# gkm2708/gym-lmaze

Hardware: AMD Instinct MI355X
Metric: env steps/sec (whole node), 1M parallel 11x11 mazes at 1/2/4/8 MI355X (higher is better)
Workload: dtype int32

## Files before the change

### gym-lmaze_amd/csrc/lmaze_foveal.hip

```cpp
#include <cstdio>
#include <cstring>
#include <type_traits>

#include "lmaze_common.h"
#include "lmaze_visit.h"

#ifdef LMAZE_EXPERIMENT
#define LMAZE_WARM_V4(args) ((((args).p.launch_hint >> 16) & 1024) != 0)
#define LMAZE_XP(args, mask) ((((args).p.launch_hint >> 16) & (mask)) != 0)
#else
#define LMAZE_WARM_V4(args) false
#define LMAZE_XP(args, mask) false
#endif

namespace lmaze {

constexpr int FOV = LMAZE_FOVEA;
constexpr int W25 = FOV * FOV;

enum FovealMode { FM_STEP = 0, FM_RESET = 1, FM_SETGOAL = 2, FM_PLANNER = 3 };

struct FovealArgs {
    LmazeFovealParams p;
    LmazeFovealBuffers b;
    const uint8_t* layouts;
    const int32_t* action;
    const int32_t* goal2;
    const uint8_t* mask;
    int64_t n;
    int32_t place;
    uint64_t seed, epoch;
    int64_t env_base;
    const uint64_t* epoch_in;
    uint64_t* epoch_out;
    int32_t nt;
    int32_t auto_reset;
    LaunchInfo* info;
};

struct FovealRoll {
    int32_t T;
    float* reward_t;
    uint8_t* done_t;
    float* freward_t;
    uint8_t* fdone_t;
};

struct FovealRollObs : FovealRoll {
    float* obs_t;
    float* obs_local_t;
    int32_t every;
};

__device__ __forceinline__ float* roll_slot(const FovealRoll&, int64_t, int64_t, int, int) { return nullptr; }
__device__ __forceinline__ float* roll_slot(const FovealRollObs& ro, int64_t n, int64_t base, int t, int per) {
    if (ro.obs_t == nullptr || (t + 1) % ro.every != 0) return nullptr;
    return ro.obs_t + ((size_t)((t + 1) / ro.every - 1) * n + base) * per;
}
__device__ __forceinline__ float* roll_lslot(const FovealRoll&, int64_t, int64_t, int) { return nullptr; }
__device__ __forceinline__ float* roll_lslot(const FovealRollObs& ro, int64_t n, int64_t base, int t) {
    if (ro.obs_local_t == nullptr || (t + 1) % ro.every != 0) return nullptr;
    return ro.obs_local_t + ((size_t)((t + 1) / ro.every - 1) * n + base) * (4 * W25);
}
__device__ __forceinline__ void roll_store4(const FovealRoll&, float4*, const float*) {}
__device__ __forceinline__ void roll_store4(const FovealRollObs&, float4* p, const float* v) {
    *p = make_float4(v[0], v[1], v[2], v[3]);
}

struct EnvRec {
    int16_t cx, cy;
    int16_t px, py;
    int16_t gx, gy;
    int16_t lid;
    int16_t action;
    int32_t skip;
    int32_t flat;
    int16_t b0x, b0y;
    int16_t b1x, b1y;
    int16_t f1x, f1y;
    int16_t upd;
    int16_t pad;
};


template <int U>
__device__ __forceinline__ void mask_counts(const uint64_t* goal_rows, const uint64_t* ball_rows, int G, int& cg, int& cb) {
    cg = 0; cb = 0;
#pragma unroll U
    for (int x = 1; x <= G - 2; ++x) { cg += __popcll(goal_rows[x]); cb += __popcll(ball_rows[x]); }
}

template <int U>
__device__ __forceinline__ int mask_kth(const uint64_t* rows, int G, int k, int hole) {
    int xr = -1, kk = 0, acc = 0;
#pragma unroll U
    for (int x = 1; x <= G - 2; ++x) {
        uint64_t m = rows[x];
        const unsigned hy = (unsigned)(hole - x * G);
        if (hy < (unsigned)G) m &= ~(1ull << hy);
        const int c = __popcll(m);
        if (xr < 0 && k < acc + c) { xr = x; kk = k - acc; }
        acc += c;
    }
    if (xr < 0) return -1;
    uint64_t m = rows[xr];
    const unsigned hy = (unsigned)(hole - xr * G);
    if (hy < (unsigned)G) m &= ~(1ull << hy);
    uint32_t h = (uint32_t)m;
    int base = 0;
    const int cl = __popc(h);
    if (kk >= cl) { kk -= cl; h = (uint32_t)(m >> 32); base = 32; }
    for (; kk > 0; --kk) h &= h - 1;
    return xr * G + base + (__ffs((int)h) - 1);
}

template <int U>
__device__ __forceinline__ void place_goal_ball(const uint64_t* goal_rows, const uint64_t* ball_rows, int G, uint4 d,
                                                int& goal_cell, int& ball_cell) {
    goal_cell = -1;
    ball_cell = -1;
    int cg, cb;
    mask_counts<U>(goal_rows, ball_rows, G, cg, cb);
    if (cg > 0) goal_cell = mask_kth<U>(goal_rows, G, (int)__umulhi(d.x, (uint32_t)cg), -1);
    if (goal_cell >= 0 && ((ball_rows[goal_cell / G] >> (goal_cell % G)) & 1ull)) --cb;
    if (cb > 0) ball_cell = mask_kth<U>(ball_rows, G, (int)__umulhi(d.y, (uint32_t)cb), goal_cell);
}

__device__ __forceinline__ int wrap5(int i) {
    if (i >= 0 && i < FOV) return i;
    if (i < 0 && i >= -FOV) return i + FOV;
    return -1;
}

__device__ __forceinline__ uint32_t window_bits(const uint64_t* rows, int G, int cx, int cy) {
    uint32_t m = 0;
    const int y0 = cy - 2;
#pragma unroll
    for (int i = 0; i < FOV; ++i) {
        const int x = cx - 2 + i;
        const uint64_t b = (x >= 0 && x < G) ? rows[x] : 0ull;
        const uint32_t w = (uint32_t)(y0 >= 0 ? (b >> y0) : (b << -y0)) & 31u;
        m |= w << (FOV * i);
    }
    return m;
}

__device__ __forceinline__ uint32_t onehot_bits(int tx, int ty, int cx, int cy) {
    const int i = tx - cx + 2, j = ty - cy + 2;
    return (i >= 0 && i < FOV && j >= 0 && j < FOV) ? (1u << (FOV * i + j)) : 0u;
}

__device__ __forceinline__ void put_bits(uint32_t* bits, int off, uint32_t m) {
    const int w = off >> 5, sh = off & 31;
    atomicOr(&bits[w], m << sh);
    if (sh > 32 - W25) atomicOr(&bits[w + 1], m >> (32 - sh));
}

__device__ __forceinline__ void lds_dma16(const uint32_t* src, uint32_t* lds_wave_base) {
    typedef __attribute__((address_space(1))) void gvoid;
    typedef __attribute__((address_space(3))) void lvoid;
    __builtin_amdgcn_global_load_lds((gvoid*)src, (lvoid*)lds_wave_base, 16, 0, 0);
}

__device__ __forceinline__ void nibble_floats(const uint32_t* bits, int q, float (&v)[4]) {
    const uint32_t nib = bits[q >> 3] >> ((q & 7) << 2);
#pragma unroll
    for (int k = 0; k < 4; ++k) v[k] = __uint_as_float((0u - ((nib >> k) & 1u)) & 0x3f800000u);
}

constexpr int VISIT_BIAS = LMAZE_VISIT_BIAS, VISIT_RENORM = LMAZE_VISIT_RENORM;
constexpr int VT = 4;
constexpr int VPC = 28;
__host__ __device__ __forceinline__ int visit_tag(int x, int y) { return 0x100 | ((x & 0x7f) << 9) | ((y & 0x7f) << 16); }

__host__ __device__ __forceinline__ int visit_tiles(int G) { return (G + VT - 1) / VT; }
__device__ __forceinline__ uint32_t visit_true(uint32_t bits, int E) { return lmaze_visit_true(bits, E); }
__device__ __forceinline__ uint32_t visit_add(uint32_t bits, int E) { return lmaze_visit_add(bits, E); }

#ifndef LMAZE_WIN_SUB
// ... 137 lines not shown
        const int row = rem / S, col = rem - row * S;
        const float* r0 = src + p * PC + (row / ET) * GT;
        const int k0 = col / ET;
        const float v0 = r0[k0], v1 = r0[k0 + 1];
        int row1 = row + 1, p1 = p;
        if (row1 == S) { row1 = 0; ++p1; }
        const float vw = src[p1 * PC + (row1 / ET) * GT];
        const int edge = (k0 + 1) * ET;
        float v[4];
#pragma unroll
        for (int j = 0; j < 4; ++j) {
            const int cj = col + j;
            v[j] = cj >= S ? vw : (cj >= edge ? v1 : v0);
        }
        const int count = len - (q << 2);
        if (count >= 4) {
            if (NT) {
                typedef float f4 __attribute__((ext_vector_type(4)));
                f4 t = {v[0], v[1], v[2], v[3]};
                stream_store16(reinterpret_cast<f4*>(dst) + q, t);
            } else {
                reinterpret_cast<float4*>(dst)[q] = make_float4(v[0], v[1], v[2], v[3]);
            }
        } else {
            for (int j = 0; j < count; ++j) dst[(q << 2) + j] = v[j];
        }
    }
}

constexpr size_t kFovealStreamBytes = (size_t)192 << 20;

static size_t lds_limit() {
    static size_t limit = 0;
    if (limit == 0) {
        int dev = 0, v = 0;
        if (hipGetDevice(&dev) == hipSuccess && hipDeviceGetAttribute(&v, hipDeviceAttributeMaxSharedMemoryPerBlock, dev) == hipSuccess && v > 0)
            limit = (size_t)v;
        else
            limit = 64 * 1024;
    }
    return limit;
}

template <int VARIANT>
static size_t foveal_lds(const LmazeFovealParams& p, int epb) {
    const int cells = p.grid * p.grid;
    const int L = VARIANT == LMAZE_VARIANT_V1 ? 1 : p.n_layouts;
    size_t lds = (size_t)epb * 64 + (3 * (size_t)L * p.grid + 2 * (size_t)p.grid) * 8 + (size_t)((L * cells + 15) & ~15);
    if (VARIANT == LMAZE_VARIANT_V4 || VARIANT == LMAZE_VARIANT_V5)
        lds += (size_t)epb * (2 * W25 * 4 + 8);
    return lds;
}

static size_t lds_for_cap(size_t lds, int per_cu) {
    if (per_cu >= 1 && per_cu <= 8) {
        const size_t cap = 160 * 1024;
        const size_t want = ((cap / per_cu + cap / (per_cu + 1)) / 2) & ~(size_t)255;
        if (want > lds && want <= lds_limit()) return want;
    }
    return lds;
}

template <int VARIANT, int MODE, int EPB>
static hipError_t launch_foveal_one(const FovealArgs& a, hipStream_t s) {
    size_t lds = foveal_lds<VARIANT>(a.p, EPB);
    if constexpr (EPB > 32) {
        if (lds > lds_limit()) return launch_foveal_one<VARIANT, MODE, EPB / 2>(a, s);
    }
    const int64_t nchunks = (a.n + EPB - 1) / EPB;
    const int m = MODE == FM_STEP ? ((a.p.launch_hint >> 8) & 3) + 1 : 1;
    const int64_t blocks = (nchunks + m - 1) / m;
    if (!grid_ok(blocks)) return hipErrorInvalidConfiguration;
    FovealArgs b = a;
    const int C = VARIANT == LMAZE_VARIANT_V1 ? 4 : (VARIANT == LMAZE_VARIANT_V2 ? 5 : 7);
    b.nt = (size_t)a.n * C * W25 * 4 > kFovealStreamBytes;
    if (LMAZE_XP(a, 2)) b.nt = 0;
    const int per_cu = a.p.launch_hint & 15;
    if (MODE == FM_STEP) lds = lds_for_cap(lds, per_cu);
    const dim3 grid((unsigned)blocks), block(LMAZE_BLOCK);
    if (a.info) {
        char name[96];
        snprintf(name, sizeof(name), "foveal_kernel<v%d, %s, %d, %d, %s>", VARIANT,
                 MODE == FM_STEP ? "step" : (MODE == FM_RESET ? "reset" : (MODE == FM_SETGOAL ? "setgoal" : "planner")), EPB,
                 (a.p.grid == 18 || a.p.grid == 14) ? a.p.grid : 0, a.auto_reset ? "fused-reset" : "plain");
        describe_launch(a.info, name, EPB, (MODE == FM_STEP && per_cu >= 1 && per_cu <= 8 && lds > (size_t)EPB * 64) ? per_cu : 0, m, b.nt != 0,
                        blocks, LMAZE_BLOCK, lds);
        return hipSuccess;
    }
    if constexpr (MODE == FM_STEP) {
        if (a.auto_reset) {
            if (a.p.grid == 18) hipLaunchKernelGGL((foveal_kernel<VARIANT, MODE, EPB, 18, true>), grid, block, lds, s, b);
            else if (a.p.grid == 14) hipLaunchKernelGGL((foveal_kernel<VARIANT, MODE, EPB, 14, true>), grid, block, lds, s, b);
            else hipLaunchKernelGGL((foveal_kernel<VARIANT, MODE, EPB, 0, true>), grid, block, lds, s, b);
            return hipGetLastError();
        }
    }
    if (a.p.grid == 18) hipLaunchKernelGGL((foveal_kernel<VARIANT, MODE, EPB, 18, false>), grid, block, lds, s, b);
    else if (a.p.grid == 14) hipLaunchKernelGGL((foveal_kernel<VARIANT, MODE, EPB, 14, false>), grid, block, lds, s, b);
    else hipLaunchKernelGGL((foveal_kernel<VARIANT, MODE, EPB, 0, false>), grid, block, lds, s, b);
    return hipGetLastError();
}

template <int VARIANT>
static bool launch_step_hinted(const FovealArgs& a, hipStream_t s, hipError_t& rc) {
    switch ((a.p.launch_hint >> 4) & 15) {
        case 2: rc = launch_foveal_one<VARIANT, FM_STEP, 32>(a, s); return true;
        case 3: rc = launch_foveal_one<VARIANT, FM_STEP, 64>(a, s); return true;
        case 4: rc = launch_foveal_one<VARIANT, FM_STEP, 128>(a, s); return true;
        case 5: rc = launch_foveal_one<VARIANT, FM_STEP, 256>(a, s); return true;
        default: return false;
    }
}

template <int MODE>
static hipError_t launch_foveal_mode(const FovealArgs& a0, hipStream_t s) {
    if (a0.n == 0) return hipSuccess;
    FovealArgs a = a0;
    if (MODE == FM_STEP && a.p.launch_hint == 0 && (!a.auto_reset || a.p.variant == LMAZE_VARIANT_V5 || a.p.variant == LMAZE_VARIANT_V6)) {
        const int C = a.p.variant == LMAZE_VARIANT_V1 ? 4 : (a.p.variant == LMAZE_VARIANT_V2 ? 5 : 7);
        if ((size_t)a.n * C * W25 * 4 > kFovealStreamBytes) {
            if (a.p.variant == LMAZE_VARIANT_V1) a.p.launch_hint = 0x220;
            else if (a.p.variant == LMAZE_VARIANT_V2) a.p.launch_hint = 0x35;
            else if (a.p.variant == LMAZE_VARIANT_V4) a.p.launch_hint = 0x140;
            else a.p.launch_hint = 0x40;
        }
    }
    if (MODE == FM_STEP && a.p.launch_hint == 0 && a.auto_reset && (size_t)a.n * W25 * 4 * 4 > kFovealStreamBytes) {
        if (a.p.variant == LMAZE_VARIANT_V1) a.p.launch_hint = 0x35;
        else if (a.p.variant == LMAZE_VARIANT_V2 || a.p.variant == LMAZE_VARIANT_V4) a.p.launch_hint = 0x140;
    }
    if (MODE == FM_STEP) {
        hipError_t rc = hipSuccess;
        switch (a.p.variant) {
            case LMAZE_VARIANT_V1: if (launch_step_hinted<LMAZE_VARIANT_V1>(a, s, rc)) return rc; break;
            case LMAZE_VARIANT_V2: if (launch_step_hinted<LMAZE_VARIANT_V2>(a, s, rc)) return rc; break;
            case LMAZE_VARIANT_V4: if (launch_step_hinted<LMAZE_VARIANT_V4>(a, s, rc)) return rc; break;
            default: if (launch_step_hinted<LMAZE_VARIANT_V5>(a, s, rc)) return rc; break;
        }
    }
    switch (a.p.variant) {
        case LMAZE_VARIANT_V1:
            if (MODE == FM_STEP && !a.auto_reset) return launch_foveal_one<LMAZE_VARIANT_V1, MODE, 32>(a, s);
            return launch_foveal_one<LMAZE_VARIANT_V1, MODE, 64>(a, s);
        case LMAZE_VARIANT_V2:
            if (MODE == FM_STEP && a.auto_reset) return launch_foveal_one<LMAZE_VARIANT_V2, MODE, 256>(a, s);
            return launch_foveal_one<LMAZE_VARIANT_V2, MODE, 64>(a, s);
        case LMAZE_VARIANT_V5:
        case LMAZE_VARIANT_V6:
            return launch_foveal_one<LMAZE_VARIANT_V5, MODE, 64>(a, s);
        default:
            if (MODE == FM_STEP && !a.auto_reset) return launch_foveal_one<LMAZE_VARIANT_V4, MODE, 32>(a, s);
            return launch_foveal_one<LMAZE_VARIANT_V4, MODE, 64>(a, s);
    }
}

template <int VARIANT, int EPB, class RO>
static hipError_t launch_rollout_one(const FovealArgs& a, const RO& ro, hipStream_t s) {
    constexpr bool REC = std::is_same<RO, FovealRollObs>::value;
    size_t lds = foveal_lds<VARIANT>(a.p, EPB);
    if constexpr (EPB > 32) {
        if (lds > lds_limit()) return launch_rollout_one<VARIANT, EPB / 2>(a, ro, s);
    }
    const int64_t nchunks = (a.n + EPB - 1) / EPB;
    const int m = ((a.p.launch_hint >> 8) & 3) + 1;
    const int64_t blocks = (nchunks + m - 1) / m;
    if (!grid_ok(blocks)) return hipErrorInvalidConfiguration;
    const int per_cu = a.p.launch_hint & 15;
    lds = lds_for_cap(lds, per_cu);
    FovealArgs b = a;
    b.nt = 0;
    constexpr int GN = VARIANT == LMAZE_VARIANT_V1 ? 14 : 18;
    const dim3 grid((unsigned)blocks), block(LMAZE_BLOCK);
    if (a.info) {
        char name[96];
        snprintf(name, sizeof(name), "foveal_rollout_kernel<v%d, %d, %d, %s%s>", VARIANT, EPB, a.p.grid == GN ? GN : 0,
                 a.auto_reset ? (VARIANT == LMAZE_VARIANT_V5 ? "two-level" : "fused-reset") : "plain", REC ? ", obs_t" : "");
        describe_launch(a.info, name, EPB, lds > foveal_lds<VARIANT>(a.p, EPB) ? per_cu : 0, m, false, blocks, LMAZE_BLOCK, lds);
        return hipSuccess;
    }
    if constexpr (VARIANT == LMAZE_VARIANT_V5) {
        if (a.p.grid == GN) hipLaunchKernelGGL((foveal_rollout_kernel<VARIANT, EPB, GN, true>), grid, block, lds, s, b, ro);
        else if constexpr (EPB == 32 && !REC) hipLaunchKernelGGL((foveal_rollout_kernel<VARIANT, 32, 0, true>), grid, block, lds, s, b, ro);
        else return hipErrorInvalidConfiguration;
    } else if constexpr (REC && VARIANT == LMAZE_VARIANT_V1) {
        if (a.p.grid != GN) return hipErrorInvalidConfiguration;
        if (a.auto_reset) hipLaunchKernelGGL((foveal_rollout_kernel<VARIANT, EPB, GN, true>), grid, block, lds, s, b, ro);
        else hipLaunchKernelGGL((foveal_rollout_kernel<VARIANT, EPB, GN, false>), grid, block, lds, s, b, ro);
    } else if (a.auto_reset) {
        if (a.p.grid == GN) hipLaunchKernelGGL((foveal_rollout_kernel<VARIANT, EPB, GN, true>), grid, block, lds, s, b, ro);
        else hipLaunchKernelGGL((foveal_rollout_kernel<VARIANT, EPB, 0, true>), grid, block, lds, s, b, ro);
    } else {
        if (a.p.grid == GN) hipLaunchKernelGGL((foveal_rollout_kernel<VARIANT, EPB, GN, false>), grid, block, lds, s, b, ro);
        else hipLaunchKernelGGL((foveal_rollout_kernel<VARIANT, EPB, 0, false>), grid, block, lds, s, b, ro);
    }
    return hipGetLastError();
}

template <int VARIANT, class RO>
static hipError_t launch_rollout_variant(const FovealArgs& a, const RO& ro, hipStream_t s) {
    if (VARIANT == LMAZE_VARIANT_V5 && a.p.grid != 18) return launch_rollout_one<VARIANT, 32>(a, ro, s);
    switch ((a.p.launch_hint >> 4) & 15) {
        case 2: return launch_rollout_one<VARIANT, 32>(a, ro, s);
        case 3: return launch_rollout_one<VARIANT, 64>(a, ro, s);
        case 4: return launch_rollout_one<VARIANT, 128>(a, ro, s);
        default: break;
    }
    if (a.n <= (int64_t)32 * 1024) return launch_rollout_one<VARIANT, 32>(a, ro, s);
    const int C = VARIANT == LMAZE_VARIANT_V1 ? 4 : (VARIANT == LMAZE_VARIANT_V2 ? 5 : 7);
    if (VARIANT != LMAZE_VARIANT_V5 && (size_t)a.n * C * W25 * 4 > kFovealStreamBytes) return launch_rollout_one<VARIANT, 128>(a, ro, s);
    return launch_rollout_one<VARIANT, 64>(a, ro, s);
}

template <class RO>
static hipError_t launch_foveal_rollout(const FovealArgs& a, const RO& ro, hipStream_t s) {
    switch (a.p.variant) {
        case LMAZE_VARIANT_V1: return launch_rollout_variant<LMAZE_VARIANT_V1>(a, ro, s);
        case LMAZE_VARIANT_V2: return launch_rollout_variant<LMAZE_VARIANT_V2>(a, ro, s);
        case LMAZE_VARIANT_V4: return launch_rollout_variant<LMAZE_VARIANT_V4>(a, ro, s);
        default: return launch_rollout_variant<LMAZE_VARIANT_V5>(a, ro, s);
    }
}

static int check_foveal(const LmazeFovealParams* p, const uint8_t* layouts, const LmazeFovealBuffers* b, int64_t n) {
    if (!p || !layouts || !b) return LMAZE_E_NULL;
// ... 382 lines not shown
```

### gym-lmaze_amd/csrc/lmaze_foveal_body.h

```cpp
#ifndef LMAZE_FOVEAL_BODY_SITE
#error "lmaze_foveal_body.h is the body of the foveal kernels: it is included only inside them, in lmaze_foveal.hip"
#endif
    constexpr bool V1 = VARIANT == LMAZE_VARIANT_V1, V5 = VARIANT == LMAZE_VARIANT_V5;
    constexpr bool V4 = VARIANT == LMAZE_VARIANT_V4 || V5;
    constexpr int C = V1 ? 4 : (V4 ? 7 : 5);
    constexpr int PLACE_U = V5 ? 1 : 4;
    constexpr int PERENV = C * W25;
    const int G = GT ? GT : a.p.grid, CELLS = G * G, L = V1 ? 1 : a.p.n_layouts;

    extern __shared__ int4 lds4[];
    uint32_t* obits = reinterpret_cast<uint32_t*>(lds4);
    uint32_t* lbits = obits + EPB * 8;
    int16_t* cen = reinterpret_cast<int16_t*>(lbits + EPB * 4);
    int32_t* flags = reinterpret_cast<int32_t*>(cen + EPB * 4);
    int16_t* rcen = reinterpret_cast<int16_t*>(flags + EPB);
    float* vwin = reinterpret_cast<float*>(rcen + EPB * 2);
    int32_t* clk = reinterpret_cast<int32_t*>(vwin + (V4 ? EPB * 2 * W25 : 0));
    int32_t* dlist = clk + (V4 ? EPB : 0);
    uint64_t* rowfree = reinterpret_cast<uint64_t*>(dlist + (V4 ? EPB : 0));
    uint64_t* rowgoal = rowfree + L * G;
    uint64_t* rowball = rowgoal + L * G;
    uint64_t* rowwall = rowball + L * G;
    uint64_t* rowx = rowwall + G;
    uint8_t* lays = reinterpret_cast<uint8_t*>(rowx + G);
    static_assert(PERENV <= 8 * 32 - 32 && 4 * W25 <= 4 * 32 - 4, "bit strings fit the 32 B / 16 B per env reserved for them");
    __shared__ int any_skip, ndense;

    const int tid = threadIdx.x;
    const int64_t nchunks = (a.n + EPB - 1) / EPB;
    int64_t chunk = blockIdx.x;
    int64_t blockbase = chunk * EPB;
    int nb = (int)min((int64_t)EPB, a.n - blockbase);
    if (tid == 0) { any_skip = 0; ndense = 0; }
    for (int i = tid; i < EPB * 12; i += LMAZE_BLOCK) obits[i] = 0u;
    if (V4) for (int i = tid; i < EPB * 2 * W25; i += LMAZE_BLOCK) vwin[i] = 0.0f;
    const uint64_t epoch = launch_epoch(a.epoch, a.epoch_in);
    if (MODE == FM_STEP && AR) pass_epoch_on(a.epoch_in, a.epoch_out);
    int warmed = 0;
    if (MODE == FM_STEP && !ROLL && a.nt) {
        warmed = warm_lines(a.action, a.n * 4, 256);
        if (!V5 || LMAZE_WARM_V4(a)) {
            warmed += warm_lines(a.b.ball_xy, a.n * 8, 256) + warm_lines(a.b.step_count, a.n * 4, 256);
            if (V1) warmed += warm_lines(a.b.fgoal_xy, a.n * 8, 256) + warm_lines(a.b.foveal_step_count, a.n * 4, 256);
            else warmed += warm_lines(a.b.goal_xy, a.n * 8, 256) + warm_lines(a.b.layout_id, a.n * 4, 256);
            if (V4) warmed += warm_lines(a.b.visit_clock, a.n * 4, 256);
            if (V5) warmed += warm_lines(a.b.fgoal_xy, a.n * 8, 256) + warm_lines(a.b.foveal_step_count, a.n * 4, 256) +
                              warm_lines(a.b.fovea_xy, a.n * 16, 256) + warm_lines(a.b.ball1_xy, a.n * 8, 256) +
                              warm_lines(a.b.last_xy, a.n * 8, 256) + warm_lines(a.b.foveal_goal, a.n * 4, 256) +
                              warm_lines(a.goal2, a.n * 4, 256);
        }
    }
    if (LMAZE_XP(a, 1)) {
    } else if (GT != 0) {
        constexpr int GG = GT ? GT : 1, RPW = 64 / GG, UNR = 8;
        const int wave = tid >> 6, lane = tid & 63, rows = L * G;
        const int rsub = lane / GG, y = lane - rsub * GG;
        const bool dwords = ((reinterpret_cast<uintptr_t>(a.layouts) | (uintptr_t)(L * CELLS)) & 3) == 0;
        uint32_t cw[2] = {0u, 0u};
        if (dwords) {
#pragma unroll
            for (int j = 0; j < 2; ++j)
                if (tid + j * LMAZE_BLOCK < (L * CELLS) >> 2) cw[j] = reinterpret_cast<const uint32_t*>(a.layouts)[tid + j * LMAZE_BLOCK];
        }
        for (int r00 = 0; r00 < rows; r00 += UNR * 4 * RPW) {
            uint8_t cc[UNR];
#pragma unroll
            for (int u = 0; u < UNR; ++u) {
                const int row = r00 + (u * 4 + wave) * RPW + rsub;
                cc[u] = (rsub < RPW && row < rows) ? a.layouts[(size_t)row * G + y] : (uint8_t)0;
            }
#pragma unroll
            for (int u = 0; u < UNR; ++u) {
                const int row = r00 + (u * 4 + wave) * RPW + rsub;
                const bool in = rsub < RPW && row < rows;
                const uint8_t c = cc[u];
                const unsigned long long bf = __ballot(in && (c == 'B' || c == 'S' || c == 'X'));
                const unsigned long long bw = __ballot(in && c == 'W');
                const unsigned long long bx = __ballot(in && c == 'X');
                const unsigned long long bs = __ballot(in && c == 'S');
                if (in && y == 0) {
                    const int sh = rsub * GG;
                    const uint64_t keep = GG == 64 ? ~0ull : ((1ull << GG) - 1ull);
                    const uint64_t fr = (bf >> sh) & keep, wl = (bw >> sh) & keep, xx = (bx >> sh) & keep, ss = (bs >> sh) & keep;
                    rowfree[row] = fr;
                    if (V1) { rowwall[row] = wl; rowx[row] = xx; }
                    if (!V1 && (MODE == FM_RESET || (MODE == FM_STEP && AR))) {
                        const int x = row % G;
                        const uint64_t interior = (x >= 1 && x <= G - 2) ? (((1ull << (G - 2)) - 1ull) << 1) : 0ull;
                        rowgoal[row] = fr & ~ss & interior;
                        rowball[row] = fr & ~xx & interior;
                    }
                }
            }
        }
        if (dwords) {
#pragma unroll
            for (int j = 0; j < 2; ++j)
                if (tid + j * LMAZE_BLOCK < (L * CELLS) >> 2) reinterpret_cast<uint32_t*>(lays)[tid + j * LMAZE_BLOCK] = cw[j];
            for (int i = tid + 2 * LMAZE_BLOCK; i < (L * CELLS) >> 2; i += LMAZE_BLOCK)
                reinterpret_cast<uint32_t*>(lays)[i] = reinterpret_cast<const uint32_t*>(a.layouts)[i];
        } else {
            for (int i = tid; i < L * CELLS; i += LMAZE_BLOCK) lays[i] = a.layouts[i];
        }
    } else {
    for (int i = tid; i < L * CELLS; i += LMAZE_BLOCK) lays[i] = a.layouts[i];
    __syncthreads();
    for (int i = tid; i < L * G; i += LMAZE_BLOCK) {
        uint64_t fr = 0, wl = 0, xx = 0;
        for (int y = 0; y < G; ++y) {
            const uint8_t c = lays[i * G + y];
            fr |= (uint64_t)(c == 'B' || c == 'S' || c == 'X') << y;
            wl |= (uint64_t)(c == 'W') << y;
            xx |= (uint64_t)(c == 'X') << y;
        }
        rowfree[i] = fr;
        if (V1) { rowwall[i] = wl; rowx[i] = xx; }
        if (!V1 && (MODE == FM_RESET || (MODE == FM_STEP && AR))) {
            uint64_t ss = 0;
            for (int y = 0; y < G; ++y) ss |= (uint64_t)(lays[i * G + y] == 'S') << y;
            const int x = i % G;
            const uint64_t interior = (x >= 1 && x <= G - 2) ? (((1ull << (G - 2)) - 1ull) << 1) : 0ull;
            rowgoal[i] = fr & ~ss & interior;
            rowball[i] = fr & ~xx & interior;
        }
    }
    }
    __syncthreads();

    int t = 0;
#define ROLL_ROW(e) (ROLL ? (int64_t)t * a.n + (e) : (e))
#define ROLL_EP (ROLL ? epoch + (uint64_t)t : epoch)
  for (;;) {
    for (int le = tid; le < (LMAZE_XP(a, 8) ? 0 : nb); le += LMAZE_BLOCK) {
        const int64_t e = blockbase + le;
        EnvRec r;
        r.skip = 0; r.flat = -1; r.action = -1; r.lid = 0; r.gx = r.gy = -9;
        r.b0x = r.b0y = r.b1x = r.b1y = r.f1x = r.f1y = 0; r.upd = 0; r.pad = 0;
        bool fresh = false, nostep = false;
        bool last_is_cur = true;
        int rx = 0, ry = 0;
        float row_r = -0.0f, row_fr = -0.0f;
        int row_d = 0, row_fd = 0;
        int bx = a.b.ball_xy[2 * e], by = a.b.ball_xy[2 * e + 1];
        const int act_in = (MODE == FM_STEP) ? a.action[ROLL_ROW(e)] : 0;
        const int sc_ld = (MODE == FM_STEP) ? a.b.step_count[e] : 0;
        const int done_in = (MODE == FM_STEP && AR) ? a.b.done[e] : 0;
        const int goal2_in = (MODE == FM_STEP && AR && V5) ? a.goal2[ROLL_ROW(e)] : 0;
        const int vword = (V4 && !(V5 && MODE == FM_PLANNER)) ? a.b.visit_clock[e] : 0;
        const int vclock = vword & 0xff;
        r.px = (int16_t)bx; r.py = (int16_t)by;
        if (MODE != FM_STEP && a.mask && !a.mask[e]) r.skip = 1;
        if (V1) {
            int fgx = a.b.fgoal_xy[2 * e], fgy = a.b.fgoal_xy[2 * e + 1];
            r.action = 1;
            if (MODE == FM_STEP) {
                int sc_in = sc_ld;
                if (AR && done_in) {
                    for (int c = 0; c < CELLS; ++c)
                        if (lays[c] == 'S') { bx = c / G; by = c % G; break; }
                    sc_in = 0;
                }
                const int act = act_in;
                const int sc = sc_in + 1;
                const int fsc = a.b.foveal_step_count[e] + 1;
                float fr = -0.0f, rw = -0.0f;
                bool local_done = false;
                int ox, oy;
                decode_action(act, ox, oy);
                const int tx = clampi(bx + ox, 0, G - 1), ty = clampi(by + oy, 0, G - 1);
                const uint8_t c = lays[tx * G + ty];
                if (c == 'W') {
                    rw = a.p.reward_wall; fr = a.p.reward_wall;
                } else if (c == 'B') {
                    bx = tx; by = ty;
                    rw = a.p.reward_move; fr = a.p.reward_move;
                    if (bx < fgx - 1 || bx > fgx + 2 || by < fgy - 1 || by > fgy + 2) {
                        local_done = true; fr = a.p.reward_wall;
                    } else if (by == fgy && bx == fgx) {
                        local_done = true; fr = a.p.reward_goal;
                    }
                } else if (c == 'X') {
                    bx = tx; by = ty;
                    rw = a.p.reward_goal;
                    if (by == fgy && bx == fgx) { local_done = true; fr = a.p.reward_goal; }
                    else fr = a.p.reward_move;
                }
                const bool done = (rw == a.p.reward_goal) || (sc == a.p.step_limit);
                const bool fdone = local_done || fr == a.p.reward_goal || fsc == a.p.foveal_step_limit || done;
                a.b.ball_xy[2 * e] = bx; a.b.ball_xy[2 * e + 1] = by;
                a.b.step_count[e] = sc; a.b.foveal_step_count[e] = fsc;
                a.b.reward[e] = rw; a.b.foveal_reward[e] = fr;
                a.b.done[e] = done ? 1 : 0; a.b.foveal_done[e] = fdone ? 1 : 0;
                row_r = rw; row_fr = fr; row_d = done; row_fd = fdone;
            } else if (MODE == FM_RESET && !r.skip) {
                if (a.place) {
                    for (int c = 0; c < CELLS; ++c)
                        if (lays[c] == 'S') { bx = c / G; by = c % G; break; }
                    a.b.ball_xy[2 * e] = bx; a.b.ball_xy[2 * e + 1] = by;
                }
                a.b.reward[e] = -0.0f; a.b.foveal_reward[e] = -0.0f;
                a.b.step_count[e] = 0;
                a.b.done[e] = 0; a.b.foveal_done[e] = 0;
                r.action = 0;
            } else if (MODE == FM_SETGOAL && !r.skip) {
                fgx = bx + a.action[2 * e] - 2;
                fgy = by + a.action[2 * e + 1] - 2;
                a.b.fgoal_xy[2 * e] = fgx; a.b.fgoal_xy[2 * e + 1] = fgy;
                a.b.foveal_step_count[e] = 0;
            }
            int flat = fgx * G + fgy;
            if (flat < 0) flat += CELLS;
            r.flat = (flat >= 0 && flat < CELLS) ? flat : -1;
        } else if (V5) {
            int lid = clampi(a.b.layout_id[e], 0, L - 1);
            int gx = a.b.goal_xy[2 * e], gy = a.b.goal_xy[2 * e + 1];
            int fg = a.b.foveal_goal[e];
            int f0x = a.b.fovea_xy[4 * e], f0y = a.b.fovea_xy[4 * e + 1];
            int f1x = a.b.fovea_xy[4 * e + 2], f1y = a.b.fovea_xy[4 * e + 3];
            int b1x = a.b.ball1_xy[2 * e], b1y = a.b.ball1_xy[2 * e + 1];
            int lx = a.b.last_xy[2 * e], ly = a.b.last_xy[2 * e + 1];
            if (MODE == FM_STEP) {
                const int act = act_in;
                int fgx = a.b.fgoal_xy[2 * e], fgy = a.b.fgoal_xy[2 * e + 1];
                int fsc = a.b.foveal_step_count[e];
                int sc_in = sc_ld;
                bool ld = a.b.foveal_done[e] != 0, gd = a.b.done[e] != 0;
                if (AR) {
                    const bool plan = ld || gd;
                    bool planned = false;
                    if (gd) {
                        const uint4 d = env_draw(a.seed, ROLL_EP, a.env_base + e);
                        lid = (int)__umulhi(d.z, (uint32_t)L);
                        int goal_cell, ball_cell;
                        place_goal_ball<PLACE_U>(rowgoal + lid * G, rowball + lid * G, G, d, goal_cell, ball_cell);
                        if (goal_cell >= 0) { gx = goal_cell / G; gy = goal_cell % G; }
                        if (ball_cell >= 0) { bx = ball_cell / G; by = ball_cell % G; }
                        a.b.layout_id[e] = lid;
                        a.b.goal_xy[2 * e] = gx; a.b.goal_xy[2 * e + 1] = gy;
                        fsc = 0; sc_in = 0; gd = false; ld = false;
                        fg = 12;
                        f0x = f1x = b1x = lx = fgx = bx; f0y = f1y = b1y = ly = fgy = by;
                        fresh = true;
                    }
                    if (plan) {
                        const int g = goal2_in;
                        if (g >= 0 && g < W25) {
                            fg = g;
                            sc_in = 0;
                            ld = false;
                            fgx = bx + g / FOV - 2; fgy = by + g % FOV - 2;
                            if (fsc > 0) { f1x = f0x; f1y = f0y; }
                            fsc += 1;
                            planned = true;
                        }
                    }
                    if (fresh || planned) {
                        a.b.foveal_goal[e] = fg;
                        a.b.fgoal_xy[2 * e] = fgx; a.b.fgoal_xy[2 * e + 1] = fgy;
                        a.b.fovea_xy[4 * e + 2] = f1x; a.b.fovea_xy[4 * e + 3] = f1y;
                        a.b.foveal_step_count[e] = fsc;
                    }
                }
                const uint8_t* lay = lays + lid * CELLS;
                b1x = bx; b1y = by;
                float lr = -0.0f, gr;
                const int sc = sc_in + 1;
                const int dx = (act == 0) - (act == 1), dy = (act == 2) - (act == 3);
                const int nx = bx + dx, ny = by + dy;
                const bool nin = nx >= 0 && ny >= 0 && nx < G && ny < G;
                const uint8_t c = nin ? lay[nx * G + ny] : (uint8_t)'W';
                if (c == 'W') {
                    lr = a.p.reward_wall;
                } else if (nx == fgx && ny == fgy) {
                    lr = a.p.reward_goal; bx = nx; by = ny; ld = true;
                } else if (c == 'B' || c == 'S' || c == 'X') {
                    if (nx < f1x - 3 || nx > f1x + 2 || ny < f1y - 3 || ny > f1y + 2) ld = true;
                    lr = a.p.reward_move; bx = nx; by = ny;
                }
                if (nx == gx && ny == gy) { gr = a.p.reward_goal; gd = true; }
                else if (nx == fgx && ny == fgy) gr = a.p.reward_move;
                else gr = a.p.reward_wall;
                f0x = bx; f0y = by;
                if (sc >= a.p.step_limit) ld = true;
                if (fsc >= a.p.foveal_step_limit) { gd = true; ld = true; }
                if (fsc == 0) { lx = f0x; ly = f0y; }
                r.px = (int16_t)lx; r.py = (int16_t)ly;
                r.upd = ld ? 1 : 0;
                if (ld) { lx = f0x; ly = f0y; }
                last_is_cur = lx == f0x && ly == f0y;
                a.b.ball_xy[2 * e] = bx; a.b.ball_xy[2 * e + 1] = by;
                a.b.ball1_xy[2 * e] = b1x; a.b.ball1_xy[2 * e + 1] = b1y;
                a.b.fovea_xy[4 * e] = f0x; a.b.fovea_xy[4 * e + 1] = f0y;
                a.b.last_xy[2 * e] = lx; a.b.last_xy[2 * e + 1] = ly;
                a.b.step_count[e] = sc;
                a.b.reward[e] = gr; a.b.foveal_reward[e] = lr;
                a.b.done[e] = gd ? 1 : 0; a.b.foveal_done[e] = ld ? 1 : 0;
                row_r = gr; row_fr = lr; row_d = gd; row_fd = ld;
            } else if (MODE == FM_PLANNER && !r.skip) {
                const int g = a.action[e];
                if (g < 0 || g >= W25) {
                    r.skip = 1;
                } else {
                    fg = g;
                    a.b.step_count[e] = 0;
                    a.b.reward[e] = -0.0f;
                    a.b.foveal_done[e] = 0;
                    a.b.foveal_goal[e] = g;
                    a.b.fgoal_xy[2 * e] = bx + g / FOV - 2;
                    a.b.fgoal_xy[2 * e + 1] = by + g % FOV - 2;
                    const int fsc = a.b.foveal_step_count[e];
                    if (fsc > 0) {
                        f1x = f0x; f1y = f0y;
                        a.b.fovea_xy[4 * e + 2] = f1x; a.b.fovea_xy[4 * e + 3] = f1y;
                    }
                    a.b.foveal_step_count[e] = fsc + 1;
                }
            } else if (MODE == FM_RESET && !r.skip) {
                if (a.place) {
                    const uint4 d = env_draw(a.seed, a.epoch, a.env_base + e);
                    lid = (int)__umulhi(d.z, (uint32_t)L);
                    a.b.layout_id[e] = lid;
                    int goal_cell, ball_cell;
                    place_goal_ball<PLACE_U>(rowgoal + lid * G, rowball + lid * G, G, d, goal_cell, ball_cell);
                    if (goal_cell >= 0) {
                        gx = goal_cell / G; gy = goal_cell % G;
                        a.b.goal_xy[2 * e] = gx; a.b.goal_xy[2 * e + 1] = gy;
                    }
                    if (ball_cell >= 0) {
                        bx = ball_cell / G; by = ball_cell % G;
                        a.b.ball_xy[2 * e] = bx; a.b.ball_xy[2 * e + 1] = by;
                    }
                }
                a.b.foveal_reward[e] = -0.0f; a.b.reward[e] = -0.0f;
                a.b.foveal_step_count[e] = 0; a.b.step_count[e] = 0;
                a.b.done[e] = 0; a.b.foveal_done[e] = 0;
                fg = 12;
                a.b.foveal_goal[e] = fg;
                f0x = f1x = b1x = lx = bx; f0y = f1y = b1y = ly = by;
                a.b.fovea_xy[4 * e] = bx; a.b.fovea_xy[4 * e + 1] = by;
                a.b.fovea_xy[4 * e + 2] = bx; a.b.fovea_xy[4 * e + 3] = by;
                a.b.fgoal_xy[2 * e] = bx; a.b.fgoal_xy[2 * e + 1] = by;
                a.b.ball1_xy[2 * e] = bx; a.b.ball1_xy[2 * e + 1] = by;
                a.b.last_xy[2 * e] = bx; a.b.last_xy[2 * e + 1] = by;
                r.px = (int16_t)bx; r.py = (int16_t)by;
            }
            r.lid = (int16_t)lid;
            r.gx = (int16_t)gx; r.gy = (int16_t)gy;
            r.action = (int16_t)fg;
            r.b0x = (int16_t)bx; r.b0y = (int16_t)by; r.b1x = (int16_t)b1x; r.b1y = (int16_t)b1y;
            r.f1x = (int16_t)f1x; r.f1y = (int16_t)f1y;
            bx = f0x; by = f0y;
        } else {
            int lid = a.b.layout_id[e];
            int gx = a.b.goal_xy[2 * e], gy = a.b.goal_xy[2 * e + 1];
            int sc_in = 0;
            const bool fused = MODE == FM_STEP && AR && done_in != 0;
            if ((MODE == FM_RESET && !r.skip) || fused) {
                if (a.place || fused) {
                    const uint4 d = env_draw(a.seed, ROLL_EP, a.env_base + e);
                    const int lid_new = (int)__umulhi(d.z, (uint32_t)L);
                    if (V4) lid = lid_new;
                    lid = clampi(lid, 0, L - 1);
                    int goal_cell, ball_cell;
                    place_goal_ball<PLACE_U>(rowgoal + lid * G, rowball + lid * G, G, d, goal_cell, ball_cell);
                    if (goal_cell >= 0) {
                        gx = goal_cell / G; gy = goal_cell % G;
                        a.b.goal_xy[2 * e] = gx; a.b.goal_xy[2 * e + 1] = gy;
                    }
                    if (ball_cell >= 0) {
                        bx = ball_cell / G; by = ball_cell % G;
                        a.b.ball_xy[2 * e] = bx; a.b.ball_xy[2 * e + 1] = by;
                    }
                    lid = lid_new;
                    a.b.layout_id[e] = lid;
                }
                a.b.reward[e] = -0.0f;
                a.b.step_count[e] = 0;
                a.b.done[e] = 0;
                r.px = (int16_t)bx; r.py = (int16_t)by;
                fresh = true;
                rx = bx; ry = by;
            } else if (MODE == FM_STEP) {
                sc_in = sc_ld;
            }
            if (MODE == FM_STEP) {
                const int act = act_in;
                if (act < 0 || act >= W25) {
                    if (fresh) nostep = true;
                    else r.skip = 1;
                    if (ROLL && !fresh) { row_r = a.b.reward[e]; row_d = a.b.done[e]; }
                } else {
                    lid = clampi(lid, 0, L - 1);
                    const uint8_t* lay = lays + lid * CELLS;
                    float rw = -0.0f;
                    const int sc = sc_in + 1;
                    const int fx = bx + act / FOV - 2, fy = by + act % FOV - 2;
                    if (fx < G - 2 && fx > 1 && fy < G - 2 && fy > 1) {
                        bx = fx; by = fy;
                    } else {
                        if (fx >= G - 2) bx = G - 3;
                        if (fx <= 1) bx = 2;
                        if (fy >= G - 2) by = G - 3;
                        if (fy <= 1) by = 2;
                    }
                    const bool fin = fx >= 0 && fy >= 0 && fx < G && fy < G;
                    const uint8_t c = fin ? lay[fx * G + fy] : (uint8_t)'W';
                    if (fx == gx && fy == gy) rw = a.p.reward_goal;
                    else if (c == 'W') rw = a.p.reward_wall;
                    else if (c == 'B' || c == 'S') rw = a.p.reward_move;
                    a.b.ball_xy[2 * e] = bx; a.b.ball_xy[2 * e + 1] = by;
                    a.b.step_count[e] = sc;
                    a.b.reward[e] = rw;
                    a.b.done[e] = (rw == a.p.reward_goal || sc > a.p.step_limit) ? 1 : 0;
                    r.action = (int16_t)act;
                    row_r = rw; row_d = rw == a.p.reward_goal || sc > a.p.step_limit;
                }
            }
// ... 69 lines not shown
    if (V4 && !(V5 && MODE == FM_PLANNER) && !LMAZE_XP(a, 32)) {
        const int TB = visit_tiles(G), TILES = TB * TB;
        uint32_t* vis = reinterpret_cast<uint32_t*>(a.b.visit) + (size_t)blockbase * TILES * (VT * VT);
        uint32_t* rec = reinterpret_cast<uint32_t*>(a.b.visit) + (size_t)a.n * TILES * (VT * VT) + (size_t)blockbase * VPC;
        auto tile_row_whole = [&](uint32_t (&s)[4], int x, int y0, int le, int fl) {
            const int E0 = clk[le];
            const bool zero = fl & 16, renorm = fl & 32, pre = fl & 64, add = fl & 128;
            const int cx = cen[le * 4], cy = cen[le * 4 + 1], px = cen[le * 4 + 2], py = cen[le * 4 + 3];
            const int E1 = zero ? 0 : (renorm ? VISIT_BIAS : E0);
            const int dx = x - cx + 2, ex = x - px + 2;
#pragma unroll 1
            for (int k = 0; k < 4; ++k) {
                const int y = y0 + k;
                const bool cell_ok = x < G && y < G;
                uint32_t b = s[k];
                if (zero) b = 0u;
                else if (renorm) b = visit_true(b, E0);
                int E = E1;
                if (pre) {
                    const int qx = x - rcen[le * 2] + 2, qy = y - rcen[le * 2 + 1] + 2;
                    if (cell_ok && (unsigned)qx <= 4u && (unsigned)qy <= 4u) b = visit_add(b, E);
                    ++E;
                }
                const int dy = y - cy + 2, ey = y - py + 2;
                const bool in = cell_ok && (unsigned)dx <= 4u && (unsigned)dy <= 4u;
                if (add) {
                    if (in) b = visit_add(b, E);
                    ++E;
                }
                s[k] = b;
                if (in) vwin[le * 2 * W25 + dx * FOV + dy] = __uint_as_float(visit_true(b, E));
                if (cell_ok && (unsigned)ex <= 4u && (unsigned)ey <= 4u)
                    vwin[le * 2 * W25 + W25 + ex * FOV + ey] = __uint_as_float(visit_true(b, E));
            }
        };
        {
            const int nd = ndense, per = TILES * VT;
            for (int j = tid; j < nd * per; j += LMAZE_BLOCK) {
                const int d = j / per, r = j - d * per;
                const int le = dlist[d], fl = flags[le];
                const int tile = r >> 2, row = r & 3;
                const int tx = tile / TB, ty = tile - tx * TB;
                uint32_t* p = vis + (le * TILES + tile) * (VT * VT) + row * VT;
                uint32_t sv[4] = {0u, 0u, 0u, 0u};
                if (!(fl & 16)) {
                    const uint4 t4 = *reinterpret_cast<const uint4*>(p);
                    sv[0] = t4.x; sv[1] = t4.y; sv[2] = t4.z; sv[3] = t4.w;
                }
                tile_row_whole(sv, tx * VT + row, ty * VT, le, fl & 0xff);
                *reinterpret_cast<uint4*>(p) = make_uint4(sv[0], sv[1], sv[2], sv[3]);
            }
        }
        {
            constexpr int IPE = 2 * FOV, SUB = EPB < LMAZE_WIN_SUB ? EPB : LMAZE_WIN_SUB, NIT = (SUB * IPE + LMAZE_BLOCK - 1) / LMAZE_BLOCK;
          for (int sb = 0; sb < nb; sb += SUB) {
            const int items = LMAZE_XP(a, 256) ? 0 : min(SUB, nb - sb) * IPE;
            uint4 va[NIT], vb[NIT];
            int meta[NIT];
#pragma unroll
            for (int u = 0; u < NIT; ++u) {
                const int i = tid + u * LMAZE_BLOCK;
                meta[u] = -1;
                va[u] = make_uint4(0u, 0u, 0u, 0u);
                vb[u] = make_uint4(0u, 0u, 0u, 0u);
                if (i >= items) continue;
                const int le = sb + i / IPE, r = i % IPE;
                const int w = r >= FOV ? 1 : 0, row = r - w * FOV;
                const int fl = flags[le];
                if (fl & (1 | 16 | 32)) continue;
                const int cx = cen[le * 4], cy = cen[le * 4 + 1];
                const int wx = cen[le * 4 + 2 * w], wy = cen[le * 4 + 2 * w + 1];
                const int x = wx - 2 + row, y0 = wy - 2;
                if ((unsigned)x >= (unsigned)G) continue;
                const bool touched = (fl & 128) && (unsigned)(x - cx + 2) <= 4u && (unsigned)(wy - cy + 4) <= 8u;
                if (V5 && w == 1 && (fl & 1024) && !touched) {
                    const int o = le * VPC + row * FOV;
                    struct __attribute__((packed, aligned(4))) Q4 { uint32_t v[4]; };
                    const Q4 q = *reinterpret_cast<const Q4*>(rec + o);
                    va[u] = make_uint4(q.v[0], q.v[1], q.v[2], q.v[3]);
                    vb[u].x = rec[o + 4];
                    meta[u] = o | (1 << 28);
                } else {
                    const int ty0 = y0 >> 2;
                    const int o = (le * TILES + (x >> 2) * TB + ty0) * (VT * VT) + (x & 3) * VT;
                    const bool a_out = ty0 < 0, b_out = ty0 + 1 >= TB;
                    if (!a_out) va[u] = *reinterpret_cast<const uint4*>(vis + o);
                    if (!b_out) vb[u] = *reinterpret_cast<const uint4*>(vis + o + VT * VT);
                    meta[u] = (o & 0x0fffffff) | (a_out ? 1 << 29 : 0) | (b_out ? 1 << 30 : 0);
                }
            }
            __syncthreads();
#pragma unroll
            for (int u = 0; u < NIT; ++u) {
                if (meta[u] < 0) continue;
                const int i = tid + u * LMAZE_BLOCK;
                const int le = sb + i / IPE, r = i % IPE;
                const int w = r >= FOV ? 1 : 0, row = r - w * FOV;
                const int fl = flags[le], E0 = clk[le];
                const bool add = fl & 128, from_rec = (meta[u] >> 28) & 1;
                const int cx = cen[le * 4], cy = cen[le * 4 + 1];
                const int x = cen[le * 4 + 2 * w] - 2 + row, y0 = cen[le * 4 + 2 * w + 1] - 2;
                const int sh = from_rec ? 0 : (y0 & 3);
                uint32_t c[8] = {va[u].x, va[u].y, va[u].z, va[u].w, vb[u].x, vb[u].y, vb[u].z, vb[u].w};
                if (sh & 1) {
#pragma unroll
                    for (int k = 0; k < 7; ++k) c[k] = c[k + 1];
                }
// ... 191 lines not shown
```

Before: 13.54 billion.

## Precompute per-layout prefix-count tables in LDS for goal/ball placement

Goal and ball placement on reset now uses per-layout cumulative popcount tables built once per block in shared memory. A vectorized row search and a branch-light kth-bit select replace the per-env loops over all rows. The LDS budget calculation subtracts the new static table so occupancy targets are kept, and the window sub-batch size is shrunk for V5 rollouts with 64 envs per block. The cost is extra shared memory and a table-build pass with an added barrier in every reset-capable block.

```diff
diff --git a/gym-lmaze_amd/csrc/lmaze_foveal.hip b/gym-lmaze_amd/csrc/lmaze_foveal.hip
--- a/gym-lmaze_amd/csrc/lmaze_foveal.hip
+++ b/gym-lmaze_amd/csrc/lmaze_foveal.hip
@@ -3,6 +3,7 @@
 #include <type_traits>
 
 #include "lmaze_common.h"
+#include "lmaze_place.h"
 #include "lmaze_visit.h"
 
 #ifdef LMAZE_EXPERIMENT
@@ -81,50 +82,6 @@
     int16_t upd;
     int16_t pad;
 };
-
-
-template <int U>
-__device__ __forceinline__ void mask_counts(const uint64_t* goal_rows, const uint64_t* ball_rows, int G, int& cg, int& cb) {
-    cg = 0; cb = 0;
-#pragma unroll U
-    for (int x = 1; x <= G - 2; ++x) { cg += __popcll(goal_rows[x]); cb += __popcll(ball_rows[x]); }
-}
-
-template <int U>
-__device__ __forceinline__ int mask_kth(const uint64_t* rows, int G, int k, int hole) {
-    int xr = -1, kk = 0, acc = 0;
-#pragma unroll U
-    for (int x = 1; x <= G - 2; ++x) {
-        uint64_t m = rows[x];
-        const unsigned hy = (unsigned)(hole - x * G);
-        if (hy < (unsigned)G) m &= ~(1ull << hy);
-        const int c = __popcll(m);
-        if (xr < 0 && k < acc + c) { xr = x; kk = k - acc; }
-        acc += c;
-    }
-    if (xr < 0) return -1;
-    uint64_t m = rows[xr];
-    const unsigned hy = (unsigned)(hole - xr * G);
-    if (hy < (unsigned)G) m &= ~(1ull << hy);
-    uint32_t h = (uint32_t)m;
-    int base = 0;
-    const int cl = __popc(h);
-    if (kk >= cl) { kk -= cl; h = (uint32_t)(m >> 32); base = 32; }
-    for (; kk > 0; --kk) h &= h - 1;
-    return xr * G + base + (__ffs((int)h) - 1);
-}
-
-template <int U>
-__device__ __forceinline__ void place_goal_ball(const uint64_t* goal_rows, const uint64_t* ball_rows, int G, uint4 d,
-                                                int& goal_cell, int& ball_cell) {
-    goal_cell = -1;
-    ball_cell = -1;
-    int cg, cb;
-    mask_counts<U>(goal_rows, ball_rows, G, cg, cb);
-    if (cg > 0) goal_cell = mask_kth<U>(goal_rows, G, (int)__umulhi(d.x, (uint32_t)cg), -1);
-    if (goal_cell >= 0 && ((ball_rows[goal_cell / G] >> (goal_cell % G)) & 1ull)) --cb;
-    if (cb > 0) ball_cell = mask_kth<U>(ball_rows, G, (int)__umulhi(d.y, (uint32_t)cb), goal_cell);
-}
 
 __device__ __forceinline__ int wrap5(int i) {
     if (i >= 0 && i < FOV) return i;
@@ -368,10 +325,17 @@
     return lds;
 }
 
-static size_t lds_for_cap(size_t lds, int per_cu) {
+template <int VARIANT>
+static size_t place_lds(bool has_reset, int gt) {
+    if (!has_reset || VARIANT == LMAZE_VARIANT_V1) return 0;
+    return (size_t)LMAZE_MAX_LAYOUTS * 2 * LMAZE_PLACE_STRIDE(gt ? gt : LMAZE_MAX_GRID) * 2;
+}
+
+static size_t lds_for_cap(size_t lds, int per_cu, size_t fixed) {
     if (per_cu >= 1 && per_cu <= 8) {
         const size_t cap = 160 * 1024;
-        const size_t want = ((cap / per_cu + cap / (per_cu + 1)) / 2) & ~(size_t)255;
+        size_t want = ((cap / per_cu + cap / (per_cu + 1)) / 2) & ~(size_t)255;
+        want = want > fixed ? want - fixed : 0;
         if (want > lds && want <= lds_limit()) return want;
     }
     return lds;
@@ -392,7 +356,7 @@
     b.nt = (size_t)a.n * C * W25 * 4 > kFovealStreamBytes;
     if (LMAZE_XP(a, 2)) b.nt = 0;
     const int per_cu = a.p.launch_hint & 15;
-    if (MODE == FM_STEP) lds = lds_for_cap(lds, per_cu);
+    if (MODE == FM_STEP) lds = lds_for_cap(lds, per_cu, place_lds<VARIANT>(a.auto_reset != 0, (a.p.grid == 18 || a.p.grid == 14) ? a.p.grid : 0));
     const dim3 grid((unsigned)blocks), block(LMAZE_BLOCK);
     if (a.info) {
         char name[96];
@@ -482,10 +446,10 @@
     const int64_t blocks = (nchunks + m - 1) / m;
     if (!grid_ok(blocks)) return hipErrorInvalidConfiguration;
     const int per_cu = a.p.launch_hint & 15;
-    lds = lds_for_cap(lds, per_cu);
+    constexpr int GN = VARIANT == LMAZE_VARIANT_V1 ? 14 : 18;
+    lds = lds_for_cap(lds, per_cu, place_lds<VARIANT>(a.auto_reset != 0, a.p.grid == GN ? GN : 0));
     FovealArgs b = a;
     b.nt = 0;
-    constexpr int GN = VARIANT == LMAZE_VARIANT_V1 ? 14 : 18;
     const dim3 grid((unsigned)blocks), block(LMAZE_BLOCK);
     if (a.info) {
         char name[96];
diff --git a/gym-lmaze_amd/csrc/lmaze_foveal_body.h b/gym-lmaze_amd/csrc/lmaze_foveal_body.h
--- a/gym-lmaze_amd/csrc/lmaze_foveal_body.h
+++ b/gym-lmaze_amd/csrc/lmaze_foveal_body.h
@@ -4,7 +4,7 @@
     constexpr bool V1 = VARIANT == LMAZE_VARIANT_V1, V5 = VARIANT == LMAZE_VARIANT_V5;
     constexpr bool V4 = VARIANT == LMAZE_VARIANT_V4 || V5;
     constexpr int C = V1 ? 4 : (V4 ? 7 : 5);
-    constexpr int PLACE_U = V5 ? 1 : 4;
+    constexpr bool HAS_RESET = MODE == FM_RESET || (MODE == FM_STEP && AR);
     constexpr int PERENV = C * W25;
     const int G = GT ? GT : a.p.grid, CELLS = G * G, L = V1 ? 1 : a.p.n_layouts;
 
@@ -23,6 +23,8 @@
     uint64_t* rowwall = rowball + L * G;
     uint64_t* rowx = rowwall + G;
     uint8_t* lays = reinterpret_cast<uint8_t*>(rowx + G);
+    constexpr int PS = LMAZE_PLACE_STRIDE(GT ? GT : LMAZE_MAX_GRID);
+    __shared__ __attribute__((aligned(16))) uint16_t ptab[(HAS_RESET && !V1) ? LMAZE_MAX_LAYOUTS * 2 * PS : 8];
     static_assert(PERENV <= 8 * 32 - 32 && 4 * W25 <= 4 * 32 - 4, "bit strings fit the 32 B / 16 B per env reserved for them");
     __shared__ int any_skip, ndense;
 
@@ -84,7 +86,7 @@
                     const uint64_t fr = (bf >> sh) & keep, wl = (bw >> sh) & keep, xx = (bx >> sh) & keep, ss = (bs >> sh) & keep;
                     rowfree[row] = fr;
                     if (V1) { rowwall[row] = wl; rowx[row] = xx; }
-                    if (!V1 && (MODE == FM_RESET || (MODE == FM_STEP && AR))) {
+                    if (!V1 && HAS_RESET) {
                         const int x = row % G;
                         const uint64_t interior = (x >= 1 && x <= G - 2) ? (((1ull << (G - 2)) - 1ull) << 1) : 0ull;
                         rowgoal[row] = fr & ~ss & interior;
@@ -115,7 +117,7 @@
         }
         rowfree[i] = fr;
         if (V1) { rowwall[i] = wl; rowx[i] = xx; }
-        if (!V1 && (MODE == FM_RESET || (MODE == FM_STEP && AR))) {
+        if (!V1 && HAS_RESET) {
             uint64_t ss = 0;
             for (int y = 0; y < G; ++y) ss |= (uint64_t)(lays[i * G + y] == 'S') << y;
             const int x = i % G;
@@ -126,6 +128,24 @@
     }
     }
     __syncthreads();
+    if (!V1 && HAS_RESET && !LMAZE_XP(a, 1)) {
+        const int ps = lmaze_place_stride(G);
+        for (int i = tid; i < L * 2 * ps; i += LMAZE_BLOCK) {
+            const int lp = i / ps, x = i - lp * ps;
+            const uint64_t* rows = ((lp & 1) ? rowball : rowgoal) + (lp >> 1) * G;
+            ptab[lp * PS + x] = lmaze_place_entry(rows, G, x);
+        }
+        __syncthreads();
+    }
+    auto place = [&](int lid, uint4 d, int& goal_cell, int& ball_cell) {
+        if (LMAZE_XP(a, 2048)) {
+            goal_cell = (1 + (int)(d.x % (unsigned)(G - 2))) * G + 1 + (int)((d.x >> 16) % (unsigned)(G - 2));
+            ball_cell = (1 + (int)(d.y % (unsigned)(G - 2))) * G + 1 + (int)((d.y >> 16) % (unsigned)(G - 2));
+            return;
+        }
+        lmaze_place_goal_ball(ptab + lid * 2 * PS, ptab + (lid * 2 + 1) * PS, rowgoal + lid * G, rowball + lid * G, G, d.x, d.y,
+                              &goal_cell, &ball_cell);
+    };
 
     int t = 0;
 #define ROLL_ROW(e) (ROLL ? (int64_t)t * a.n + (e) : (e))
@@ -232,7 +252,7 @@
                         const uint4 d = env_draw(a.seed, ROLL_EP, a.env_base + e);
                         lid = (int)__umulhi(d.z, (uint32_t)L);
                         int goal_cell, ball_cell;
-                        place_goal_ball<PLACE_U>(rowgoal + lid * G, rowball + lid * G, G, d, goal_cell, ball_cell);
+                        place(lid, d, goal_cell, ball_cell);
                         if (goal_cell >= 0) { gx = goal_cell / G; gy = goal_cell % G; }
                         if (ball_cell >= 0) { bx = ball_cell / G; by = ball_cell % G; }
                         a.b.layout_id[e] = lid;
@@ -321,7 +341,7 @@
                     lid = (int)__umulhi(d.z, (uint32_t)L);
                     a.b.layout_id[e] = lid;
                     int goal_cell, ball_cell;
-                    place_goal_ball<PLACE_U>(rowgoal + lid * G, rowball + lid * G, G, d, goal_cell, ball_cell);
+                    place(lid, d, goal_cell, ball_cell);
                     if (goal_cell >= 0) {
                         gx = goal_cell / G; gy = goal_cell % G;
                         a.b.goal_xy[2 * e] = gx; a.b.goal_xy[2 * e + 1] = gy;
@@ -362,7 +382,7 @@
                     if (V4) lid = lid_new;
                     lid = clampi(lid, 0, L - 1);
                     int goal_cell, ball_cell;
-                    place_goal_ball<PLACE_U>(rowgoal + lid * G, rowball + lid * G, G, d, goal_cell, ball_cell);
+                    place(lid, d, goal_cell, ball_cell);
                     if (goal_cell >= 0) {
                         gx = goal_cell / G; gy = goal_cell % G;
                         a.b.goal_xy[2 * e] = gx; a.b.goal_xy[2 * e + 1] = gy;
@@ -538,7 +558,7 @@
             }
         }
         {
-            constexpr int IPE = 2 * FOV, SUB = EPB < LMAZE_WIN_SUB ? EPB : LMAZE_WIN_SUB, NIT = (SUB * IPE + LMAZE_BLOCK - 1) / LMAZE_BLOCK;
+            constexpr int IPE = 2 * FOV, SUB = (REC && V5 && EPB == 64) ? 32 : (EPB < LMAZE_WIN_SUB ? EPB : LMAZE_WIN_SUB), NIT = (SUB * IPE + LMAZE_BLOCK - 1) / LMAZE_BLOCK;
           for (int sb = 0; sb < nb; sb += SUB) {
             const int items = LMAZE_XP(a, 256) ? 0 : min(SUB, nb - sb) * IPE;
             uint4 va[NIT], vb[NIT];
diff --git a/gym-lmaze_amd/csrc/lmaze_place.h b/gym-lmaze_amd/csrc/lmaze_place.h
--- /dev/null
+++ b/gym-lmaze_amd/csrc/lmaze_place.h
@@ -0,0 +1,87 @@
+#ifndef LMAZE_PLACE_H_
+#define LMAZE_PLACE_H_
+
+#include <stdint.h>
+
+#ifndef LMAZE_HD
+#ifdef __HIPCC__
+#define LMAZE_HD __host__ __device__ __forceinline__
+#else
+#define LMAZE_HD static inline
+#endif
+#endif
+
+typedef struct __attribute__((aligned(16))) { uint32_t w[4]; } lmaze_place_vec;
+
+#define LMAZE_PLACE_STRIDE(G) (((G) + 1 + 7) & ~7)
+LMAZE_HD int lmaze_place_stride(int G) { return LMAZE_PLACE_STRIDE(G); }
+
+LMAZE_HD uint16_t lmaze_place_entry(const uint64_t* rows, int G, int x) {
+    int acc = 0;
+    for (int r = 0; r < G; ++r) {
+        const int c = __builtin_popcountll(rows[r]);
+        acc += r < x ? c : 0;
+    }
+    return x <= G ? (uint16_t)acc : (uint16_t)0xffffu;
+}
+
+LMAZE_HD uint32_t lmaze_place_mulhi(uint32_t a, uint32_t b) { return (uint32_t)(((uint64_t)a * b) >> 32); }
+
+LMAZE_HD int lmaze_place_row(const uint16_t* cum, int G, int k) {
+    const lmaze_place_vec* v = (const lmaze_place_vec*)cum;
+    const int nv = lmaze_place_stride(G) >> 3;
+    int n = 0;
+#ifdef __clang__
+#pragma unroll 1
+#endif
+    for (int i = 0; i < nv; ++i) {
+        const lmaze_place_vec q = v[i];
+        for (int j = 0; j < 4; ++j)
+            n += ((int)(q.w[j] & 0xffffu) <= k ? 1 : 0) + ((int)(q.w[j] >> 16) <= k ? 1 : 0);
+    }
+    return n - 1;
+}
+
+LMAZE_HD int lmaze_place_kth_bit(uint64_t m, int k) {
+    uint32_t h = (uint32_t)m;
+    int pos = 0;
+    int c = __builtin_popcount(h);
+    if (k >= c) { k -= c; h = (uint32_t)(m >> 32); pos = 32; }
+    for (int s = 16; s >= 1; s >>= 1) {
+        const uint32_t lo = h & ((1u << s) - 1u);
+        c = __builtin_popcount(lo);
+        const int up = k >= c ? 1 : 0;
+        k -= up ? c : 0;
+        h = up ? h >> s : lo;
+        pos += up ? s : 0;
+    }
+    return pos;
+}
+
+LMAZE_HD void lmaze_place_goal_ball(const uint16_t* cum_goal, const uint16_t* cum_ball, const uint64_t* goal_rows,
+                                    const uint64_t* ball_rows, int G, uint32_t dx, uint32_t dy, int* goal_cell, int* ball_cell) {
+    *goal_cell = -1;
+    *ball_cell = -1;
+    const int cg = cum_goal[G];
+    int cb = cum_ball[G];
+    int rg = -1;
+    if (cg > 0) {
+        const int kg = (int)lmaze_place_mulhi(dx, (uint32_t)cg);
+        const int gx = lmaze_place_row(cum_goal, G, kg);
+        const int gy = lmaze_place_kth_bit(goal_rows[gx], kg - cum_goal[gx]);
+        *goal_cell = gx * G + gy;
+        const uint64_t b = ball_rows[gx];
+        if ((b >> gy) & 1ull) {
+            rg = cum_ball[gx] + __builtin_popcountll(b & ((1ull << gy) - 1ull));
+            --cb;
+        }
+    }
+    if (cb > 0) {
+        int kb = (int)lmaze_place_mulhi(dy, (uint32_t)cb);
+        if (rg >= 0 && kb >= rg) ++kb;
+        const int bx = lmaze_place_row(cum_ball, G, kb);
+        *ball_cell = bx * G + lmaze_place_kth_bit(ball_rows[bx], kb - cum_ball[bx]);
+    }
+}
+
+#endif
```

After: 13.65 billion, median of 3. No clear change (+0.8%).
